# peterdavidfagan/mujoco_robot_environments

Measured on AMD Instinct MI355X. Metric: env steps/sec (whole node), RearrangementEnv batch=4096 at 1/2/4/8 MI355X, higher is better.
Workload: dtype f32

## Files before the change

mujoco_robot_environments_amd/csrc/mre_kernels.hip:

```cpp
#include <hip/hip_runtime.h>

#include "mre_dev.h"
#include "mre_math.h"
#include "mre_collide.h"

namespace mre {
using ModelP = MRE_MODEL_PTR(DevModel);
#if defined(MRE_PHASE_STAMPS) && MRE_PHASE_STAMPS >= 4
__shared__ unsigned long long dbg_acc[4];
#endif

struct OscSm {
  float J[6][7], M[7][7], MiJt[7][6], Li[6][6], Lam[6][6], V[6][6], Jbar[7][6];
  float ep[3], eo[3], F[6], LF[6], tn[7], Jbt[6], xd[6], w[6];
};

struct alignas(8) Blk {
  uint16_t row0;
  uint8_t type, nrows;
  uint8_t rslot;
  uint8_t pa, pb;
  uint8_t primary : 4;
  uint8_t bslot : 4;
};
// ... 1043 lines not shown
        if (ten >= 0) v -= h * grip_bias2 * ten_coef * ten_coef;
      }
    }
    mh_store(s)[e] = v;
#ifdef MRE_NEWTON
    if (i == j) s.scratch[i] = (s.qM[e] - v) * s.qacc[i];
#endif
  }
#ifndef MRE_NEWTON
  if (l < NRV) s.scratch[l] = s.qfrc_smooth[l] + s.qfrc_con[l];
#endif
  MRE_SYNC();
}

MRE_DEV void q_store(float* p, float v) {
  __hip_atomic_store(reinterpret_cast<int*>(p), __float_as_int(v), __ATOMIC_RELAXED, __HIP_MEMORY_SCOPE_AGENT);
}
MRE_DEV void q_store(int* p, int v) { __hip_atomic_store(p, v, __ATOMIC_RELAXED, __HIP_MEMORY_SCOPE_AGENT); }
template <bool WT>
MRE_DEV void travel_store(float* p, float v) {
  if (WT) q_store(p, v); else *p = v;
}
typedef unsigned q_u32x4 __attribute__((ext_vector_type(4)));
MRE_DEV void q_store_row(float* row, const float* src, int n, int l, bool zero_last = false) {
  const __amdgpu_buffer_rsrc_t rsrc = __builtin_amdgcn_make_buffer_rsrc(row, 0, n * 4, 0x00020000);
  if (4 * l < n) {
    q_u32x4 v;
    v.x = __float_as_uint(src[4 * l]); v.y = __float_as_uint(src[4 * l + 1]); v.z = __float_as_uint(src[4 * l + 2]);
    v.w = zero_last && 4 * l + 4 == n ? 0u : __float_as_uint(src[4 * l + 3]);
    __builtin_amdgcn_raw_buffer_store_b128(v, rsrc, 16 * l, 0, 16 );
  }
}

template <bool WT>
MRE_PHASE_FN void integrate(ModelP M, Sm& s, int l, unsigned flags, bool polished, float* clo) {
  const float h = M->opt_rec.timestep;
  const auto* DR = &M->dof_rec[l < NV ? l : 0];
  const int dof_b = DR->body, dof_pid = DR->propid;
  const auto* BR = &M->body_rec[l < NB ? l : 0];
  const int body_qa = BR->qposadr, body_da = BR->dofadr, body_pid = BR->propid;
  const bool freeze = (flags & F_FREEZE_ROBOT) != 0;
  float vl_in = 0.f, ql_in[7] = {0.f, 0.f, 0.f, 0.f, 0.f, 0.f, 0.f};
  if (clo != nullptr) {
    if (l >= NRV && l < NV) vl_in = clo[(QFINE_CUBE_V - QFINE_CUBE_Q) + (l - NRV)];
    if (l >= NRB && l < NB) {
#pragma unroll
      for (int k = 0; k < 7; k++) ql_in[k] = clo[7 * (l - NRB) + k];
    }
  }
  keep_live(dof_pid); keep_live(body_pid); keep_live(body_qa); keep_live(body_da);
  if (l < NV) {
    const int b = dof_b;
    if (b < NRB) {
      if (!freeze) {
#ifdef MRE_NEWTON
        const double acc = polished ? reinterpret_cast<const double*>(&s.nw_Mv[0])[l] : (double)s.qacc[l];
        const double v = robot_v(s, l) + (double)h * (acc + (double)s.scratch[l]);
#else
        const double v = robot_v(s, l) + (double)h * (double)s.scratch[l];
#endif
        const float hi = (float)v;
        s.qvel[l] = hi; s.qlo[QFINE / 2 + l] = (float)(v - (double)hi);
      }
    } else if (prop_is_active(s, dof_pid)) {
      if (clo != nullptr) {
        float* const vl = clo + (QFINE_CUBE_V - QFINE_CUBE_Q) + (l - NRV);
        const double v = (double)s.qvel[l] + (double)vl_in + (double)h * (double)s.qacc[l];
        const float hi = (float)v, lo = (float)(v - (double)hi);
        s.qvel[l] = hi; travel_store<WT>(vl, lo);
        s.scratch[l] = lo;
      } else {
        s.qvel[l] += h * s.qacc[l];
      }
    }
  }
  MRE_SYNC();
  if (l >= 1 && l < NB) {
    const int b = l, qa = body_qa, da = body_da;
    if (b < NRB) {
      if (!freeze) {
        const double q = robot_q(s, qa) + (double)h * robot_v(s, da);
        const float hi = (float)q;
        s.qpos[qa] = hi; s.qlo[qa] = (float)(q - (double)hi);
      }
    } else if (prop_is_active(s, body_pid) && clo != nullptr) {
      float* const ql = clo + 7 * (b - NRB);
      double vv[6];
      for (int k = 0; k < 6; k++) vv[k] = (double)s.qvel[da + k] + (double)s.scratch[da + k];
      for (int k = 0; k < 3; k++) {
        const double x = (double)s.qpos[qa + k] + (double)ql_in[k] + (double)h * vv[k];
        const float hi = (float)x;
        s.qpos[qa + k] = hi; travel_store<WT>(ql + k, (float)(x - (double)hi));
      }
      double q0[4], qn[4];
      for (int k = 0; k < 4; k++) q0[k] = (double)s.qpos[qa + 3 + k] + (double)ql_in[3 + k];
      const double wn2 = vv[3] * vv[3] + vv[4] * vv[4] + vv[5] * vv[5];
      if (wn2 > 1e-60) {
        const double inv = rsq64(wn2), half = 0.5 * (double)h * wn2 * inv;
        double sn, cs;
        sincos_poly_d(half, sn, cs);
        const double ax = vv[3] * inv * sn, ay = vv[4] * inv * sn, az = vv[5] * inv * sn;
        qn[0] = q0[0] * cs - q0[1] * ax - q0[2] * ay - q0[3] * az;
        qn[1] = q0[0] * ax + q0[1] * cs + q0[2] * az - q0[3] * ay;
        qn[2] = q0[0] * ay - q0[1] * az + q0[2] * cs + q0[3] * ax;
        qn[3] = q0[0] * az + q0[1] * ay - q0[2] * ax + q0[3] * cs;
      } else {
        for (int k = 0; k < 4; k++) qn[k] = q0[k];
      }
      const double nn = qn[0] * qn[0] + qn[1] * qn[1] + qn[2] * qn[2] + qn[3] * qn[3];
      const double sc = nn > 1e-30 ? rsq64(nn) : 1.0;
      for (int k = 0; k < 4; k++) {
        const double x = qn[k] * sc;
        const float hi = (float)x;
        s.qpos[qa + 3 + k] = hi; travel_store<WT>(ql + 3 + k, (float)(x - (double)hi));
      }
    } else if (prop_is_active(s, body_pid)) {
      for (int k = 0; k < 3; k++) s.qpos[qa + k] += h * s.qvel[da + k];
      float w[3] = {s.qvel[da + 3], s.qvel[da + 4], s.qvel[da + 5]};
      const float ang = v3normalize(w) * h;
      float qr[4], qn[4], q0[4];
      axisangle2q(qr, w, ang);
      for (int k = 0; k < 4; k++) q0[k] = s.qpos[qa + 3 + k];
      qmul(qn, q0, qr);
      qnormalize(qn);
      for (int k = 0; k < 4; k++) s.qpos[qa + 3 + k] = qn[k];
    }
  }
  MRE_SYNC();
}

#ifdef MRE_PHASE_STAMPS
#define MRE_STAMP(k)                                                         \
  do {                                                                       \
    if ((k) < 12 || MRE_PHASE_STAMPS == 3) {                                 \
      const unsigned long long now_ = __builtin_amdgcn_s_memtime();          \
      if ((k) / 4 == MRE_PHASE_STAMPS) stamp_acc[(k) % 4] += now_ - stamp_t; \
      stamp_t = now_;                                                        \
    }                                                                        \
  } while (0)
#else
#define MRE_STAMP(k) do {} while (0)
#endif

MRE_DEV int q_load(const int* p) { return __hip_atomic_load(p, __ATOMIC_RELAXED, __HIP_MEMORY_SCOPE_AGENT); }

#ifdef MRE_LARGE_CAPS
constexpr bool Q_LARGE = true;
#else
constexpr bool Q_LARGE = false;
#endif
MRE_DEV int* q_bucket(const StepArgs& a, int t, int sh) {
  const int S = a.q_shards;
  return a.q_buf + (size_t)t * a.q_stride + (sh < S ? (size_t)sh * a.q_cap : (size_t)S * a.q_cap + (size_t)(sh - S) * a.q_capl);
}

MRE_DEV int queue_pop_shard(const StepArgs& a, int l, int sh, int& env, int& tick) {
  const int S = a.q_shards;
  const bool order0 = sh < S;
  const int n0 = (a.N - sh + S - 1) / S;
  int* const head = a.q_head + sh * QUEUE_TICKS_MAX;
  const int* const tail = a.q_tail + sh * QUEUE_TICKS_MAX;
  for (;;) {
    int h[QUEUE_TICKS_MAX / 64], tl[QUEUE_TICKS_MAX / 64];
#pragma unroll
    for (int c = 0; c < QUEUE_TICKS_MAX / 64; c++) {
      const int b = c * 64 + l;
      h[c] = 0; tl[c] = 0;
      if (b < a.q_nticks) { h[c] = q_load(head + b); tl[c] = (b == 0 && order0) ? n0 : q_load(tail + b); }
    }
    int t = -1, ht = 0;
#pragma unroll
    for (int c = 0; c < QUEUE_TICKS_MAX / 64; c++) {
      if (t < 0 && c * 64 < a.q_nticks) {
        const unsigned long long ready = __ballot(h[c] < tl[c]);
        if (ready != 0ull) {
          const int k = __ffsll((long long)ready) - 1;
          t = c * 64 + k;
          ht = __builtin_amdgcn_readlane(h[c], k);
        }
      }
    }
    if (t < 0) return 0;
    int got = -1;
    if (l == 0) {
      if (t == 0 && order0) {
        const int i = __hip_atomic_fetch_add(head, 1, __ATOMIC_RELAXED, __HIP_MEMORY_SCOPE_AGENT);
        if (i < n0) got = a.env_order != nullptr ? a.env_order[sh + S * i] : sh + S * i;
      } else {
        int expect = ht;
        if (__hip_atomic_compare_exchange_strong(head + t, &expect, ht + 1, __ATOMIC_RELAXED, __ATOMIC_RELAXED,
                                                 __HIP_MEMORY_SCOPE_AGENT)) {
          const int* slot = q_bucket(a, t, sh) + ht;
          int v = q_load(slot);
          for (unsigned spin = 0; v == 0; ++spin) {
            if (spin > (1u << 20)) { *a.q_err = 1; v = -1; break; }
            __builtin_amdgcn_s_sleep(4);
            v = q_load(slot);
          }
          got = v < 0 ? -2 : v - 1;
        }
      }
    }
    got = __builtin_amdgcn_readfirstlane(got);
    if (got == -2) return -1;
    if (got < 0) continue;
    env = got; tick = t;
    return 1;
  }
}
MRE_DEV bool queue_pop(const StepArgs& a, int l, int home, int& env, int& tick, int& shard, bool wait = true) {
  const int S = a.q_shards;
  if (Q_LARGE) {
    const int SL = a.q_lshards;
    for (unsigned idle = 0;; ++idle) {
      int r = 0;
      for (int k = 0; k < SL && r == 0; ++k) {
        const int sh = S + (home + k < SL ? home + k : home + k - SL);
        r = queue_pop_shard(a, l, sh, env, tick);
        if (r != 0) shard = sh;
      }
      if (r != 0) return r > 0;
      if (!wait || a.q_wait == 0 || q_load(a.q_done) >= a.N) return false;
      if (idle > 512u && q_load(a.q_started) == 0) return false;
      if (idle > (1u << 18)) return false;
      __builtin_amdgcn_s_sleep(127);
    }
  }
  for (int k = 0; k < S; ++k) {
    const int sh = home + k < S ? home + k : home + k - S;
    const int r = queue_pop_shard(a, l, sh, env, tick);
    if (r != 0) { shard = sh; return r > 0; }
  }
  return false;
}
#ifdef MRE_NEWTON
constexpr bool Q_WRITE_THROUGH = true;
#else
constexpr bool Q_WRITE_THROUGH = false;
#endif
MRE_DEV void queue_push(const StepArgs& a, int l, int env, int tick, int shard) {
  if (!Q_WRITE_THROUGH) __builtin_amdgcn_fence(__ATOMIC_RELEASE, "agent");
  asm volatile("s_waitcnt vmcnt(0)" ::: "memory");
  if (l == 0) {
    const int i = __hip_atomic_fetch_add(a.q_tail + shard * QUEUE_TICKS_MAX + tick, 1, __ATOMIC_RELAXED, __HIP_MEMORY_SCOPE_AGENT);
    __hip_atomic_store(q_bucket(a, tick, shard) + i, env + 1, __ATOMIC_RELAXED, __HIP_MEMORY_SCOPE_AGENT);
  }
}

struct QueueItem {
  bool have = false;
  int env = 0, tick = 0, shard = 0, nprops = 0;
  float qpos = 0.f, qvel = 0.f, qacc = 0.f, qfine = 0.f, ctrl = 0.f, prop_size = 0.f;
};
#ifdef MRE_NEWTON
constexpr bool Q_EARLY_TAKE = true;
#else
constexpr bool Q_EARLY_TAKE = false;
#endif
MRE_DEV void queue_take(const StepArgs& a, int l, int home, bool wait, QueueItem& it) {
  it.have = queue_pop(a, l, home, it.env, it.tick, it.shard, wait);
  if (!it.have) return;
  if (it.tick > 0 || Q_LARGE) __builtin_amdgcn_fence(__ATOMIC_ACQUIRE, "agent");
  const size_t e = (size_t)it.env;
  it.qpos = l < NQP ? a.qpos[e * NQP + l] : 0.f;
  it.qvel = l < NVP ? a.qvel[e * NVP + l] : 0.f;
  it.qacc = l < NVP ? a.qacc_ws[e * NVP + l] : 0.f;
  it.qfine = l < QFINE && a.qfine != nullptr ? a.qfine[e * QFINE_ROW + l] : 0.f;
  it.ctrl = l < NU ? a.ctrl[e * NU + l] : 0.f;
  it.prop_size = l < NPROP * 3 ? a.prop_size[e * NPROP * 3 + l] : 0.f;
  it.nprops = a.nprops[e];
}

template <bool QUEUE>
MRE_DEV void step_body(const StepArgs& a, Sm& s) {
  OscSm& osc = s.osc;
  const int l = threadIdx.x;
  int env = 0, qtick = 0, qshard = 0;
  if (!QUEUE) {
    if ((int)blockIdx.x >= a.N) return;
    env = a.env_order != nullptr ? a.env_order[blockIdx.x] : (int)blockIdx.x;
  }
  if (QUEUE && !Q_LARGE && l == 0) __hip_atomic_fetch_add(a.q_started, 1, __ATOMIC_RELAXED, __HIP_MEMORY_SCOPE_AGENT);
  if (QUEUE && Q_LARGE && a.q_wait != 0) {
    for (unsigned idle = 0; q_load(a.q_gen) != a.q_gen_expect; ++idle) {
      if (idle > 1024u) return;
      __builtin_amdgcn_s_sleep(127);
    }
  }
  const int qhome = QUEUE ? (int)(blockIdx.x % (unsigned)(Q_LARGE ? a.q_lshards : a.q_shards)) : 0;
  QueueItem next;
 for (;;) {
  if (QUEUE) {
    if (!next.have) queue_take(a, l, qhome, true, next);
    if (!next.have) return;
    env = next.env; qtick = next.tick; qshard = next.shard;
    next.have = false;
  }
  const int step_lo = QUEUE ? qtick * a.control_steps : 0, step_hi = QUEUE ? step_lo + a.control_steps : a.nsteps;
  if (QUEUE && !Q_LARGE && qtick == 0 && a.large != nullptr && a.large[env] != 0) continue;
  if (!QUEUE || (!Q_LARGE && qtick == 0)) {
#define MRE_PASS_SKIP { if (QUEUE) { if (l == 0) __hip_atomic_fetch_add(a.q_done, 1, __ATOMIC_RELAXED, __HIP_MEMORY_SCOPE_AGENT); continue; } return; }
  if (!QUEUE && a.large != nullptr && (a.large[env] != 0) != (a.want_large != 0)) return;
  if (a.env_mask != nullptr && a.env_mask[env] == 0) {
    if (a.launch_info != nullptr && l < 4) a.launch_info[(size_t)env * 4 + l] = -1;
    MRE_PASS_SKIP;
  }
  if (a.pending != nullptr && a.pending[env] != 0) {
    if (a.launch_info != nullptr && l < 4) a.launch_info[(size_t)env * 4 + l] = l == 0 ? -2 : -1;
    MRE_PASS_SKIP;
  }
#undef MRE_PASS_SKIP
  }
  ModelP M = (ModelP)a.M;

  const bool save = !QUEUE && a.sv_qpos != nullptr && step_lo == 0;
  if (l < NQP) {
    const float v = QUEUE ? next.qpos : a.qpos[(size_t)env * NQP + l];
    s.qpos[l] = v;
    if (save) a.sv_qpos[(size_t)env * NQP + l] = v;
  }
  if (l < NVP) {
    const float v = QUEUE ? next.qvel : a.qvel[(size_t)env * NVP + l], w = QUEUE ? next.qacc : a.qacc_ws[(size_t)env * NVP + l];
    s.qvel[l] = v;
    s.qacc[l] = w;
    s.qfrc_con[l] = 0.f;
    if (save) { a.sv_qvel[(size_t)env * NVP + l] = v; a.sv_qacc_ws[(size_t)env * NVP + l] = w; }
  }
  if (l < QFINE) {
    const float v = QUEUE ? next.qfine : a.qfine != nullptr ? a.qfine[(size_t)env * QFINE_ROW + l] : 0.f;
    s.qlo[l] = v;
    if (save && a.qfine != nullptr) a.sv_qfine[(size_t)env * QFINE_ROW + l] = v;
  }
  if (save && a.qfine != nullptr && l < QFINE_ROW - QFINE)
    a.sv_qfine[(size_t)env * QFINE_ROW + QFINE + l] = a.qfine[(size_t)env * QFINE_ROW + QFINE + l];
  float cube_lo_keep = 0.f;
  if (QUEUE && !Q_LARGE && a.qfine != nullptr && l < QFINE_ROW - QFINE) cube_lo_keep = a.qfine[(size_t)env * QFINE_ROW + QFINE + l];
  if (l < NU) {
    const float v = QUEUE ? next.ctrl : a.ctrl[(size_t)env * NU + l];
    s.ctrl[l] = v;
    if (save) a.sv_ctrl[(size_t)env * NU + l] = v;
  }
  if (save && l == 0) {
    if (a.nstep != nullptr) a.sv_nstep[env] = a.nstep[env];
    a.sv_status[env] = a.status[env];
    a.sv_converged[env] = a.converged != nullptr ? a.converged[env] : (uint8_t)0;
  }
  if (l == 0) { s.nprops = QUEUE ? next.nprops : a.nprops[env]; s.overflow = 0; s.ncon = 0; s.nefc = 0; s.solver_iters = 0; }
#ifdef MRE_NEWTON
  if (l < 24) s.zrow[l] = 0.f;
#endif
  if (l < NPROP * 3) {
    const float sz = QUEUE ? next.prop_size : a.prop_size[(size_t)env * NPROP * 3 + l];
    s.prop_size[l / 3][l % 3] = sz;
  }
  MRE_SYNC();
  if (l < NPROP) {
    const float m = M->body_mass[NRB + l];
    const float* z = s.prop_size[l];
    s.prop_mass[l] = m;
    s.prop_inertia[l][0] = m / 3.f * (z[1] * z[1] + z[2] * z[2]);
    s.prop_inertia[l][1] = m / 3.f * (z[0] * z[0] + z[2] * z[2]);
    s.prop_inertia[l][2] = m / 3.f * (z[0] * z[0] + z[1] * z[1]);
  }
  MRE_SYNC();

#if defined(MRE_PHASE_STAMPS) && MRE_PHASE_STAMPS >= 4
  if (l < 4) dbg_acc[l] = 0ull;
#endif
#ifdef MRE_PHASE_STAMPS
  unsigned long long stamp_acc[4] = {0, 0, 0, 0};
  unsigned long long stamp_t = __builtin_amdgcn_s_memtime();
#endif
  bool arm_converged = ((a.flags & F_CONV_CONTINUE) != 0 || (QUEUE && qtick > 0)) && a.converged != nullptr && a.converged[env] != 0;
  float grip_cmd = 0.f;
  const OscConfig* oscp = a.osc + (size_t)env * a.osc_stride;
  int hw_ncon = 0, hw_nefc = 0, hw_nrrow = 0, hw_npp = 0;
  const unsigned long long launch_t0 = __builtin_amdgcn_s_memtime();
  if (a.mode == CTRL_OSC) {
    if (l < 16) s.osc_tgt[l] = a.osc_target[(size_t)env * 16 + l];
    grip_cmd = a.grip_closed[env] ? M->act_ctrlrange[NU - 1][1] : M->act_ctrlrange[NU - 1][0];
    MRE_SYNC();
  }
  int steps_done = 0;
  bool settled = false;
  for (int step = step_lo; step < step_hi; ++step) {
    MRE_STAMP(7);
    position_stage(M, s, l);
    MRE_STAMP(12);
    MRE_STAMP(13);
    gripper_local(M, s, l);
    if ((a.flags & F_NO_CONSTRAINTS) == 0) connect_rows_local(M, s, l);
    MRE_STAMP(14);
    crb_mass_matrix(M, s, l);
    MRE_SYNC();
#ifndef MRE_NEWTON
    factor_robot_regs(s.qM, s.qLD, s.qLDinv);
#endif
    MRE_STAMP(15);
    MRE_STAMP(0);

    velocity_stage(M, s, l);
    MRE_SYNC();
    finger_bias(M, s, l);
    MRE_STAMP(1);
    const bool constrained = (a.flags & F_NO_CONSTRAINTS) == 0;
    if (constrained) {

      collide(M, s, l, false, (a.flags & F_CLIP_ALWAYS) != 0);
      MRE_STAMP(2);
      assemble_constraints(M, s, l);
#ifdef MRE_NEWTON
      nw_build_lists(s, l, a.flags);
#else
      solve_robot_rows(s, l);
      assemble_blocks(M, s, l);
#endif
      MRE_STAMP(3);
      hw_ncon = max(hw_ncon, s.ncon); hw_nefc = max(hw_nefc, s.nefc);
      hw_nrrow = max(hw_nrrow, s.nrrow); hw_npp = max(hw_npp, s.npp);
    }

    if (a.mode == CTRL_SEQ && (step % a.control_steps) == 0) {
      const int tick = step / a.control_steps;
      if (l < NU) s.ctrl[l] = a.ctrl_seq[((size_t)tick * a.seq_stride + env) * NU + l];
      MRE_SYNC();
    }
    if (a.mode == CTRL_OSC && (step % a.control_steps) == 0) {
      if (step > 0 && osc_converged(M, s, oscp, s.osc_tgt)) arm_converged = true;
      osc_compute(M, s, osc, oscp, s.osc_tgt, l);
      if (l == 0) s.ctrl[NU - 1] = grip_cmd;
      MRE_SYNC();
    }
    MRE_STAMP(4);
    const unsigned clamped = smooth_forces(M, s, l);
    MRE_STAMP(5);
    bool polished = false;
    if (constrained) {
#if defined(MRE_NEWTON) && defined(MRE_PHASE_STAMPS)
      newton_solve(M, s, l, stamp_acc, stamp_t);
      polished = nw_robot_polish(M, s, l);
#elif defined(MRE_NEWTON)
      newton_solve(M, s, l);
      polished = nw_robot_polish(M, s, l);
#else
      if (M->opt_rec.cone == 0) solve_constraints_pyramidal(M, s, l);
      else solve_constraints(M, s, l);
#endif
      MRE_STAMP(6);
    } else {
      if (l < NVP) { s.qacc[l] = s.qacc_smooth[l]; s.qfrc_con[l] = 0.f; }
      MRE_SYNC();
    }

    if (QUEUE && Q_EARLY_TAKE && step + 1 == step_hi) queue_take(a, l, qhome, false, next);
    float cube_lo_warm = 0.f;
    if (QUEUE && Q_WRITE_THROUGH && a.qfine != nullptr && l < QFINE_ROW - QFINE) cube_lo_warm = a.qfine[(size_t)env * QFINE_ROW + QFINE + l];
    integrate_setup(M, s, l, clamped);
    factor_solve_robot(mh_store(s), s.scratch, l);
    if (QUEUE && Q_WRITE_THROUGH) keep_live(cube_lo_warm);
    integrate<QUEUE && Q_WRITE_THROUGH>(M, s, l, a.flags, polished, a.qfine != nullptr ? a.qfine + (size_t)env * QFINE_ROW + QFINE_CUBE_Q : nullptr);
    steps_done = step + 1 - step_lo;
    if ((a.flags & F_SETTLE_EXIT) != 0) {
      float mv = 0.f, ma = 0.f;
      if (l >= NRV && l < NRV + 6 * s.nprops) { mv = fabsf(s.qvel[l]); ma = fabsf(s.qacc[l]); }
      mv = wave_max(mv); ma = wave_max(ma);
      settled = mv < 1e-3f && ma < 1e-2f && step + 1 > a.min_settle_steps;
    }
    if (a.trace != nullptr && env < a.trace_nenv && (a.trace_base + step) < a.trace_max) {
      if (l < TRACE_QVEL) {
        float v = l < NQ ? s.qpos[l] : 0.f;
        if (l == NQ && constrained) {
          int mask = 0;
          for (int k = 0; k < s.nl; k++) mask |= 1 << ((s.lim_info[k] & 0xFF) - 1);
          v = (float)(s.ncon + 64 * mask);
        }
        if (l == NQ + 1 && constrained) {
          unsigned h = 0u;
          for (int c = 0; c < s.ncon; c++) {
            const int pr = s.con_pair[c];
            const unsigned key = (unsigned)(M->pair_g1[pr] * 32 + M->pair_g2[pr] + 1);
            h = (h + key * key) & 0x3FFFFFu;
          }
          v = (float)h;
        }
        if (l == NQ + 2 && constrained && M->opt_rec.cone != 0) {
          unsigned h = 0u;
          const int ns = 7 + s.nl;
          for (int i = 7; i < ns; i++) h += (s.frc[i] > 0.f ? 1u : 2u) * (unsigned)((i + 1) * (i + 1));
          for (int c = 0; c < s.ncon; c++) {
            const int i = ns + 3 * c;
#ifdef MRE_NEWTON
            const float mu = s.con_fric[c];
#else
            const float mu = s.blkrec[8 + c][15];
#endif
            const float fn = s.frc[i], ft2 = s.frc[i + 1] * s.frc[i + 1] + s.frc[i + 2] * s.frc[i + 2], lim = mu * fn;
            const unsigned z = fn <= 0.f ? 1u : (ft2 >= lim * lim * (1.f - 1e-4f) ? 3u : 2u);
            h += z * (unsigned)((c + 3) * (c + 3));
          }
          v = (float)(h & 0x3FFFFFu);
        }
        travel_store<QUEUE && Q_WRITE_THROUGH>(&a.trace[((size_t)(a.trace_base + step) * a.trace_nenv + env) * TRACE_W + l], v);
      }
      if (l < NVP)
        travel_store<QUEUE && Q_WRITE_THROUGH>(&a.trace[((size_t)(a.trace_base + step) * a.trace_nenv + env) * TRACE_W + TRACE_QVEL + l],
                                               l < NV ? s.qvel[l] : 0.f);
    }
    if (settled) break;
  }
  MRE_STAMP(7);
  if (a.settle_steps != nullptr && l == 0) a.settle_steps[env] = settled ? steps_done : -steps_done;
  const bool hand_over = QUEUE && !Q_LARGE && s.overflow != 0;
  if (QUEUE && Q_WRITE_THROUGH) {
    if (hand_over) {
      if (a.qfine != nullptr && l < QFINE_ROW - QFINE) q_store(a.qfine + (size_t)env * QFINE_ROW + QFINE + l, cube_lo_keep);
    } else {
      q_store_row(a.qpos + (size_t)env * NQP, s.qpos, NQP, l);
      q_store_row(a.qvel + (size_t)env * NVP, s.qvel, NVP, l);
      q_store_row(a.qacc_ws + (size_t)env * NVP, s.qacc, NVP, l, true);
      if (a.qfine != nullptr) q_store_row(a.qfine + (size_t)env * QFINE_ROW, s.qlo, QFINE, l);
      q_store_row(a.ctrl + (size_t)env * NU, s.ctrl, NU, l);
    }
  }
  if (a.nstep != nullptr && l == 0 && !hand_over) {
    if (QUEUE) __hip_atomic_fetch_add(a.nstep + env, steps_done, __ATOMIC_RELAXED, __HIP_MEMORY_SCOPE_AGENT);
    else a.nstep[env] += steps_done;
  }
  if (a.nsteps == 0 && (a.flags & F_OSC_EVAL) != 0 && a.mode == CTRL_OSC) {
    position_stage(M, s, l);
    gripper_local(M, s, l);
    crb_mass_matrix(M, s, l);
    MRE_SYNC();
    velocity_stage(M, s, l);
    MRE_SYNC();
    osc_compute(M, s, osc, oscp, s.osc_tgt, l);
    if (l == 0) s.ctrl[NU - 1] = grip_cmd;
    MRE_SYNC();
  }
  if (a.nsteps == 0 && (a.flags & F_DETECT) != 0 && a.contacts != nullptr) {
    position_stage(M, s, l);
    collide(M, s, l, (a.flags & F_DETECT_ACTIVE) == 0, (a.flags & F_CLIP_ALWAYS) != 0);
    float* o = a.contacts + (size_t)env * (1 + 3 * CONTACT_EXPORT);
    const int n = s.ncon < CONTACT_EXPORT ? s.ncon : CONTACT_EXPORT;
    if (l == 0) o[0] = s.overflow ? -(float)s.ncon : (float)s.ncon;
    if (l < n) {
      const int pr = s.con_pair[l];
      o[1 + 3 * l] = (float)M->pair_g1[pr]; o[2 + 3 * l] = (float)M->pair_g2[pr]; o[3 + 3 * l] = s.con_dist[l];
      if (a.contacts_full != nullptr) {
        float* f = a.contacts_full + ((size_t)env * CONTACT_EXPORT + l) * 12;
        for (int k = 0; k < 3; k++) f[k] = s.con_pos[l][k];
        for (int k = 0; k < 9; k++) f[3 + k] = s.con_frame[l][k];
      }
    }
    MRE_SYNC();
    if (l == 0) s.overflow = 0;
  }
  const bool q_last = !QUEUE || (qtick + 1 == a.q_nticks && !hand_over);
  if (q_last && (a.mode == CTRL_OSC || a.sites != nullptr || a.geoms != nullptr)) kinematics_only(M, s, l);
  if (a.mode == CTRL_OSC && a.nsteps > 0 && !hand_over) {
    if (q_last && osc_converged(M, s, oscp, s.osc_tgt)) arm_converged = true;
    if (l == 0) {
      if (a.converged != nullptr) {
        if (QUEUE && Q_WRITE_THROUGH) __hip_atomic_store(a.converged + env, (uint8_t)(arm_converged ? 1 : 0), __ATOMIC_RELAXED, __HIP_MEMORY_SCOPE_AGENT);
        else a.converged[env] = arm_converged ? 1 : 0;
      }
      if (q_last && !arm_converged && a.status != nullptr && (a.flags & F_CONV_OPEN) == 0) {
        if (QUEUE) __hip_atomic_fetch_or(a.status + env, 1u, __ATOMIC_RELAXED, __HIP_MEMORY_SCOPE_AGENT);
        else a.status[env] |= 1u;
      }
    }
  }
  if (a.geoms != nullptr && l < NG) {
    float p[3], R[9], size[3], rb;
    geom_pose(M, s, l, p, R, size, &rb);
    float* o = a.geoms + ((size_t)env * NG + l) * 16;
    const int pid = M->geom_propid[l];
    const bool active = pid < 0 || pid < s.nprops;
    for (int k = 0; k < 3; k++) o[k] = p[k];
    for (int k = 0; k < 9; k++) o[3 + k] = R[k];
    for (int k = 0; k < 3; k++) o[12 + k] = size[k];
    o[15] = active ? (float)M->geom_type[l] : -1.f;
  }
  if (a.sites != nullptr && q_last) {
    float* o = a.sites + (size_t)env * 16;
    if (l < 3) o[l] = s.site_xpos[M->opt_rec.tcp_site][l];
    if (l >= 3 && l < 6) o[l] = s.site_xpos[M->opt_rec.eef_site][l - 3];
    if (l == 6) {
      float q[4];
      mat2q(q, s.site_xmat[0]);
      o[6] = q[0]; o[7] = q[1]; o[8] = q[2]; o[9] = q[3];
    }
  }
  if (QUEUE && Q_WRITE_THROUGH) {
  } else if (hand_over) {
    if (a.qfine != nullptr && l < QFINE_ROW - QFINE) a.qfine[(size_t)env * QFINE_ROW + QFINE + l] = cube_lo_keep;
  } else {
    if (l < NQP) a.qpos[(size_t)env * NQP + l] = s.qpos[l];
    if (l < NVP) {
      a.qvel[(size_t)env * NVP + l] = s.qvel[l];
      a.qacc_ws[(size_t)env * NVP + l] = l < NV ? s.qacc[l] : 0.f;
    }
    if (l < QFINE && a.qfine != nullptr) a.qfine[(size_t)env * QFINE_ROW + l] = s.qlo[l];
    if (l < NU) a.ctrl[(size_t)env * NU + l] = s.ctrl[l];
  }
  const bool q_more = QUEUE && !hand_over && qtick + 1 < a.q_nticks;
  if (l == 0 && a.launch_info != nullptr) {
    int* li = a.launch_info + (size_t)env * 4;
    unsigned long long dt = (__builtin_amdgcn_s_memtime() - launch_t0) >> 10;
    int moved = 0;
    if (QUEUE) {
      int* qa = a.q_acc + (size_t)env * 4;
      if (qtick > 0 || Q_LARGE) {
        hw_ncon = max(hw_ncon, q_load(qa + 0) & 0xFFFF); hw_nefc = max(hw_nefc, q_load(qa + 1));
        hw_nrrow = max(hw_nrrow, q_load(qa + 2) & 0xFFFF); hw_npp = max(hw_npp, q_load(qa + 2) >> 16);
        dt += (unsigned long long)q_load(qa + 3);
        moved = q_load(qa + 0) >> 16;
      }
      if (hand_over) moved = 1;
      if ((q_more || hand_over) && Q_WRITE_THROUGH) {
        q_store(qa + 0, hw_ncon | (moved << 16)); q_store(qa + 1, hw_nefc); q_store(qa + 2, hw_nrrow | (hw_npp << 16)); q_store(qa + 3, (int)dt);
      } else if (q_more || hand_over) {
        qa[0] = hw_ncon | (moved << 16); qa[1] = hw_nefc; qa[2] = hw_nrrow | (hw_npp << 16); qa[3] = (int)dt;
      }
      else dt /= (unsigned long long)(qtick + 1);
    }
    if (!q_more && !hand_over) {
#ifdef MRE_LARGE_CAPS
      li[0] = (s.overflow ? 2 : 0) | (moved ? 4 : 0);
#else
      li[0] = s.overflow ? 1 : 0;
#endif
      li[1] = hw_ncon | ((int)(dt < 0x7FFFull ? dt : 0x7FFFull) << 16); li[2] = hw_nefc; li[3] = hw_nrrow | (hw_npp << 16);
    }
  }
#ifndef MRE_LARGE_CAPS
  if (!QUEUE && l == 0 && a.pending != nullptr && s.overflow) a.pending[env] = 1;
#endif
  if (l == 0 && a.status != nullptr && !hand_over) {
    unsigned st = 0;
    for (int k = 0; k < NQ; k++) if (!isfinite(s.qpos[k])) st |= 2u;
    if (s.overflow) st |= 4u;
    if (QUEUE) { if (st) __hip_atomic_fetch_or(a.status + env, st, __ATOMIC_RELAXED, __HIP_MEMORY_SCOPE_AGENT); }
    else a.status[env] |= st;
    if (a.stats != nullptr && a.nsteps > 0 && !(QUEUE && Q_WRITE_THROUGH && q_more)) {
      a.stats[env * 4 + 0] = s.ncon; a.stats[env * 4 + 1] = s.nefc;
      a.stats[env * 4 + 2] = s.solver_iters; a.stats[env * 4 + 3] = s.nl;
#ifdef MRE_PHASE_STAMPS
      for (int k = 0; k < 4; k++) a.stats[env * 4 + k] = (int)(stamp_acc[k] >> 4);
#if MRE_PHASE_STAMPS >= 4
      for (int k = 0; k < 4; k++) a.stats[env * 4 + k] = (int)(dbg_acc[k] >> 4);
#endif
#endif
    }
  }
  if (!QUEUE) return;
  if (hand_over) queue_push(a, l, env, qtick, a.q_shards + env % a.q_lshards);
  else if (q_more) queue_push(a, l, env, qtick + 1, qshard);
  else if (l == 0) __hip_atomic_fetch_add(a.q_done, 1, __ATOMIC_RELAXED, __HIP_MEMORY_SCOPE_AGENT);
 }
}

#ifdef MRE_NEWTON
#define MRE_VARIANT(name) name##_newton
#else
#define MRE_VARIANT(name) name
#endif

#ifdef MRE_LARGE_CAPS
__global__ __launch_bounds__(64, 2) void MRE_VARIANT(k_step_large)(StepArgs a) {
  __shared__ Sm s;
  step_body<false>(a, s);
}
}

extern "C" void MRE_VARIANT(mre_launch_step_large)(const mre::StepArgs* args, hipStream_t stream) {
  hipLaunchKernelGGL(mre::MRE_VARIANT(k_step_large), dim3(args->N), dim3(64), 0, stream, *args);
}
namespace mre {
__global__ __launch_bounds__(64, 2) void MRE_VARIANT(k_step_queue_large)(StepArgs a) {
  __shared__ Sm s;
  step_body<true>(a, s);
}
}
extern "C" void MRE_VARIANT(mre_launch_step_queue_large)(const mre::StepArgs* args, int nwaves, hipStream_t stream) {
  hipLaunchKernelGGL(mre::MRE_VARIANT(k_step_queue_large), dim3(nwaves), dim3(64), 0, stream, *args);
}
#else
__global__ __launch_bounds__(64, 2) void MRE_VARIANT(k_step)(StepArgs a) {
  __shared__ Sm s;
  step_body<false>(a, s);
}
// ... 366 lines not shown
```

Measured before the change: 25.99 million.

## Load cold kernel args lazily and keep cube low words in LDS, not global

Rarely used StepArgs fields are now read on demand from the kernarg segment through volatile loads, so the compiler stops holding them in scalar registers across the long step loop. The cubes' low-order position and velocity words are kept in a register per lane and staged through shared memory borrowed from the constraint block during integration. This replaces the per-step global or atomic write-through to qfine, which is now written once at the end. The aim is to cut SGPR pressure and per-step global traffic. The cost is extra kernarg reloads at the use sites and an added barrier in integrate.

```diff
diff --git a/mujoco_robot_environments_amd/csrc/mre_kernels.hip b/mujoco_robot_environments_amd/csrc/mre_kernels.hip
--- a/mujoco_robot_environments_amd/csrc/mre_kernels.hip
+++ b/mujoco_robot_environments_amd/csrc/mre_kernels.hip
@@ -1099,8 +1099,14 @@
   }
 }
 
-template <bool WT>
-MRE_PHASE_FN void integrate(ModelP M, Sm& s, int l, unsigned flags, bool polished, float* clo) {
+MRE_DEV float* cube_lo_room(Sm& s) { return &s.JpA[0][0]; }
+static_assert(sizeof(((Sm*)0)->JpA) >= sizeof(float) * (QFINE_ROW - QFINE) && QFINE_ROW - QFINE <= 64, "the cubes' low words fit the head of the constraint block, one per lane");
+MRE_PHASE_FN float integrate(ModelP M, Sm& s, int l, unsigned flags, bool polished, bool have_lo, float cube_lo) {
+  float* const clo = cube_lo_room(s);
+  if (have_lo) {
+    if (l < QFINE_ROW - QFINE) clo[l] = cube_lo;
+    MRE_SYNC();
+  }
   const float h = M->opt_rec.timestep;
   const auto* DR = &M->dof_rec[l < NV ? l : 0];
   const int dof_b = DR->body, dof_pid = DR->propid;
@@ -1108,7 +1114,7 @@
   const int body_qa = BR->qposadr, body_da = BR->dofadr, body_pid = BR->propid;
   const bool freeze = (flags & F_FREEZE_ROBOT) != 0;
   float vl_in = 0.f, ql_in[7] = {0.f, 0.f, 0.f, 0.f, 0.f, 0.f, 0.f};
-  if (clo != nullptr) {
+  if (have_lo) {
     if (l >= NRV && l < NV) vl_in = clo[(QFINE_CUBE_V - QFINE_CUBE_Q) + (l - NRV)];
     if (l >= NRB && l < NB) {
 #pragma unroll
@@ -1130,11 +1136,11 @@
         s.qvel[l] = hi; s.qlo[QFINE / 2 + l] = (float)(v - (double)hi);
       }
     } else if (prop_is_active(s, dof_pid)) {
-      if (clo != nullptr) {
+      if (have_lo) {
         float* const vl = clo + (QFINE_CUBE_V - QFINE_CUBE_Q) + (l - NRV);
         const double v = (double)s.qvel[l] + (double)vl_in + (double)h * (double)s.qacc[l];
         const float hi = (float)v, lo = (float)(v - (double)hi);
-        s.qvel[l] = hi; travel_store<WT>(vl, lo);
+        s.qvel[l] = hi; *vl = lo;
         s.scratch[l] = lo;
       } else {
         s.qvel[l] += h * s.qacc[l];
@@ -1150,14 +1156,14 @@
         const float hi = (float)q;
         s.qpos[qa] = hi; s.qlo[qa] = (float)(q - (double)hi);
       }
-    } else if (prop_is_active(s, body_pid) && clo != nullptr) {
+    } else if (prop_is_active(s, body_pid) && have_lo) {
       float* const ql = clo + 7 * (b - NRB);
       double vv[6];
       for (int k = 0; k < 6; k++) vv[k] = (double)s.qvel[da + k] + (double)s.scratch[da + k];
       for (int k = 0; k < 3; k++) {
         const double x = (double)s.qpos[qa + k] + (double)ql_in[k] + (double)h * vv[k];
         const float hi = (float)x;
-        s.qpos[qa + k] = hi; travel_store<WT>(ql + k, (float)(x - (double)hi));
+        s.qpos[qa + k] = hi; ql[k] = (float)(x - (double)hi);
       }
       double q0[4], qn[4];
       for (int k = 0; k < 4; k++) q0[k] = (double)s.qpos[qa + 3 + k] + (double)ql_in[3 + k];
@@ -1179,7 +1185,7 @@
       for (int k = 0; k < 4; k++) {
         const double x = qn[k] * sc;
         const float hi = (float)x;
-        s.qpos[qa + 3 + k] = hi; travel_store<WT>(ql + 3 + k, (float)(x - (double)hi));
+        s.qpos[qa + 3 + k] = hi; ql[3 + k] = (float)(x - (double)hi);
       }
     } else if (prop_is_active(s, body_pid)) {
       for (int k = 0; k < 3; k++) s.qpos[qa + k] += h * s.qvel[da + k];
@@ -1194,6 +1200,8 @@
     }
   }
   MRE_SYNC();
+  if (have_lo && l < QFINE_ROW - QFINE) cube_lo = clo[l];
+  return cube_lo;
 }
 
 #ifdef MRE_PHASE_STAMPS
@@ -1211,6 +1219,18 @@
 
 MRE_DEV int q_load(const int* p) { return __hip_atomic_load(p, __ATOMIC_RELAXED, __HIP_MEMORY_SCOPE_AGENT); }
 
+#if defined(__HIP_DEVICE_COMPILE__)
+template <class T>
+MRE_DEV T cold_arg(size_t off) {
+  const char __attribute__((address_space(4)))* seg = (const char __attribute__((address_space(4)))*)__builtin_amdgcn_kernarg_segment_ptr();
+  return *(const volatile T __attribute__((address_space(4)))*)(seg + off);
+}
+#else
+template <class T>
+MRE_DEV T cold_arg(size_t) { return T(); }
+#endif
+#define MRE_COLD(member) cold_arg<decltype(StepArgs::member)>(offsetof(StepArgs, member))
+
 #ifdef MRE_LARGE_CAPS
 constexpr bool Q_LARGE = true;
 #else
@@ -1252,7 +1272,7 @@
     if (l == 0) {
       if (t == 0 && order0) {
         const int i = __hip_atomic_fetch_add(head, 1, __ATOMIC_RELAXED, __HIP_MEMORY_SCOPE_AGENT);
-        if (i < n0) got = a.env_order != nullptr ? a.env_order[sh + S * i] : sh + S * i;
+        if (i < n0) { const int* const order = MRE_COLD(env_order); got = order != nullptr ? order[sh + S * i] : sh + S * i; }
       } else {
         int expect = ht;
         if (__hip_atomic_compare_exchange_strong(head + t, &expect, ht + 1, __ATOMIC_RELAXED, __ATOMIC_RELAXED,
@@ -1260,7 +1280,7 @@
           const int* slot = q_bucket(a, t, sh) + ht;
           int v = q_load(slot);
           for (unsigned spin = 0; v == 0; ++spin) {
-            if (spin > (1u << 20)) { *a.q_err = 1; v = -1; break; }
+            if (spin > (1u << 20)) { *MRE_COLD(q_err) = 1; v = -1; break; }
             __builtin_amdgcn_s_sleep(4);
             v = q_load(slot);
           }
@@ -1287,8 +1307,8 @@
         if (r != 0) shard = sh;
       }
       if (r != 0) return r > 0;
-      if (!wait || a.q_wait == 0 || q_load(a.q_done) >= a.N) return false;
-      if (idle > 512u && q_load(a.q_started) == 0) return false;
+      if (!wait || MRE_COLD(q_wait) == 0 || q_load(MRE_COLD(q_done)) >= a.N) return false;
+      if (idle > 512u && q_load(MRE_COLD(q_started)) == 0) return false;
       if (idle > (1u << 18)) return false;
       __builtin_amdgcn_s_sleep(127);
     }
@@ -1317,7 +1337,7 @@
 struct QueueItem {
   bool have = false;
   int env = 0, tick = 0, shard = 0, nprops = 0;
-  float qpos = 0.f, qvel = 0.f, qacc = 0.f, qfine = 0.f, ctrl = 0.f, prop_size = 0.f;
+  float qpos = 0.f, qvel = 0.f, qacc = 0.f, qfine = 0.f, cube_lo = 0.f, ctrl = 0.f, prop_size = 0.f;
 };
 #ifdef MRE_NEWTON
 constexpr bool Q_EARLY_TAKE = true;
@@ -1333,6 +1353,7 @@
   it.qvel = l < NVP ? a.qvel[e * NVP + l] : 0.f;
   it.qacc = l < NVP ? a.qacc_ws[e * NVP + l] : 0.f;
   it.qfine = l < QFINE && a.qfine != nullptr ? a.qfine[e * QFINE_ROW + l] : 0.f;
+  it.cube_lo = l < QFINE_ROW - QFINE && a.qfine != nullptr ? a.qfine[e * QFINE_ROW + QFINE + l] : 0.f;
   it.ctrl = l < NU ? a.ctrl[e * NU + l] : 0.f;
   it.prop_size = l < NPROP * 3 ? a.prop_size[e * NPROP * 3 + l] : 0.f;
   it.nprops = a.nprops[e];
@@ -1345,11 +1366,14 @@
   int env = 0, qtick = 0, qshard = 0;
   if (!QUEUE) {
     if ((int)blockIdx.x >= a.N) return;
-    env = a.env_order != nullptr ? a.env_order[blockIdx.x] : (int)blockIdx.x;
-  }
-  if (QUEUE && !Q_LARGE && l == 0) __hip_atomic_fetch_add(a.q_started, 1, __ATOMIC_RELAXED, __HIP_MEMORY_SCOPE_AGENT);
-  if (QUEUE && Q_LARGE && a.q_wait != 0) {
-    for (unsigned idle = 0; q_load(a.q_gen) != a.q_gen_expect; ++idle) {
+    const int* const order = MRE_COLD(env_order);
+    env = order != nullptr ? order[blockIdx.x] : (int)blockIdx.x;
+  }
+  if (QUEUE && !Q_LARGE && l == 0) __hip_atomic_fetch_add(MRE_COLD(q_started), 1, __ATOMIC_RELAXED, __HIP_MEMORY_SCOPE_AGENT);
+  if (QUEUE && Q_LARGE && MRE_COLD(q_wait) != 0) {
+    const int* const gen = MRE_COLD(q_gen);
+    const int gen_expect = MRE_COLD(q_gen_expect);
+    for (unsigned idle = 0; q_load(gen) != gen_expect; ++idle) {
       if (idle > 1024u) return;
       __builtin_amdgcn_s_sleep(127);
     }
@@ -1364,53 +1388,67 @@
     next.have = false;
   }
   const int step_lo = QUEUE ? qtick * a.control_steps : 0, step_hi = QUEUE ? step_lo + a.control_steps : a.nsteps;
-  if (QUEUE && !Q_LARGE && qtick == 0 && a.large != nullptr && a.large[env] != 0) continue;
+  if (QUEUE && !Q_LARGE && qtick == 0) {
+    const uint8_t* const large = MRE_COLD(large);
+    if (large != nullptr && large[env] != 0) continue;
+  }
   if (!QUEUE || (!Q_LARGE && qtick == 0)) {
-#define MRE_PASS_SKIP { if (QUEUE) { if (l == 0) __hip_atomic_fetch_add(a.q_done, 1, __ATOMIC_RELAXED, __HIP_MEMORY_SCOPE_AGENT); continue; } return; }
-  if (!QUEUE && a.large != nullptr && (a.large[env] != 0) != (a.want_large != 0)) return;
-  if (a.env_mask != nullptr && a.env_mask[env] == 0) {
-    if (a.launch_info != nullptr && l < 4) a.launch_info[(size_t)env * 4 + l] = -1;
+#define MRE_PASS_SKIP { if (QUEUE) { if (l == 0) __hip_atomic_fetch_add(MRE_COLD(q_done), 1, __ATOMIC_RELAXED, __HIP_MEMORY_SCOPE_AGENT); continue; } return; }
+  if (!QUEUE) {
+    const uint8_t* const large = MRE_COLD(large);
+    if (large != nullptr && (large[env] != 0) != (MRE_COLD(want_large) != 0)) return;
+  }
+  const uint8_t* const env_mask = MRE_COLD(env_mask);
+  if (env_mask != nullptr && env_mask[env] == 0) {
+    int* const info = MRE_COLD(launch_info);
+    if (info != nullptr && l < 4) info[(size_t)env * 4 + l] = -1;
     MRE_PASS_SKIP;
   }
-  if (a.pending != nullptr && a.pending[env] != 0) {
-    if (a.launch_info != nullptr && l < 4) a.launch_info[(size_t)env * 4 + l] = l == 0 ? -2 : -1;
+  const uint8_t* const pending = MRE_COLD(pending);
+  if (pending != nullptr && pending[env] != 0) {
+    int* const info = MRE_COLD(launch_info);
+    if (info != nullptr && l < 4) info[(size_t)env * 4 + l] = l == 0 ? -2 : -1;
     MRE_PASS_SKIP;
   }
 #undef MRE_PASS_SKIP
   }
   ModelP M = (ModelP)a.M;
 
-  const bool save = !QUEUE && a.sv_qpos != nullptr && step_lo == 0;
+  const bool save = !QUEUE && MRE_COLD(sv_qpos) != nullptr && step_lo == 0;
   if (l < NQP) {
     const float v = QUEUE ? next.qpos : a.qpos[(size_t)env * NQP + l];
     s.qpos[l] = v;
-    if (save) a.sv_qpos[(size_t)env * NQP + l] = v;
+    if (save) MRE_COLD(sv_qpos)[(size_t)env * NQP + l] = v;
   }
   if (l < NVP) {
     const float v = QUEUE ? next.qvel : a.qvel[(size_t)env * NVP + l], w = QUEUE ? next.qacc : a.qacc_ws[(size_t)env * NVP + l];
     s.qvel[l] = v;
     s.qacc[l] = w;
     s.qfrc_con[l] = 0.f;
-    if (save) { a.sv_qvel[(size_t)env * NVP + l] = v; a.sv_qacc_ws[(size_t)env * NVP + l] = w; }
+    if (save) { MRE_COLD(sv_qvel)[(size_t)env * NVP + l] = v; MRE_COLD(sv_qacc_ws)[(size_t)env * NVP + l] = w; }
   }
   if (l < QFINE) {
     const float v = QUEUE ? next.qfine : a.qfine != nullptr ? a.qfine[(size_t)env * QFINE_ROW + l] : 0.f;
     s.qlo[l] = v;
-    if (save && a.qfine != nullptr) a.sv_qfine[(size_t)env * QFINE_ROW + l] = v;
-  }
-  if (save && a.qfine != nullptr && l < QFINE_ROW - QFINE)
-    a.sv_qfine[(size_t)env * QFINE_ROW + QFINE + l] = a.qfine[(size_t)env * QFINE_ROW + QFINE + l];
-  float cube_lo_keep = 0.f;
-  if (QUEUE && !Q_LARGE && a.qfine != nullptr && l < QFINE_ROW - QFINE) cube_lo_keep = a.qfine[(size_t)env * QFINE_ROW + QFINE + l];
+    if (save && a.qfine != nullptr) MRE_COLD(sv_qfine)[(size_t)env * QFINE_ROW + l] = v;
+  }
+  const bool have_lo = a.qfine != nullptr;
+  float cube_lo = 0.f;
+  if (l < QFINE_ROW - QFINE && have_lo) {
+    cube_lo = QUEUE ? next.cube_lo : a.qfine[(size_t)env * QFINE_ROW + QFINE + l];
+    if (save) MRE_COLD(sv_qfine)[(size_t)env * QFINE_ROW + QFINE + l] = cube_lo;
+  }
   if (l < NU) {
     const float v = QUEUE ? next.ctrl : a.ctrl[(size_t)env * NU + l];
     s.ctrl[l] = v;
-    if (save) a.sv_ctrl[(size_t)env * NU + l] = v;
+    if (save) MRE_COLD(sv_ctrl)[(size_t)env * NU + l] = v;
   }
   if (save && l == 0) {
-    if (a.nstep != nullptr) a.sv_nstep[env] = a.nstep[env];
-    a.sv_status[env] = a.status[env];
-    a.sv_converged[env] = a.converged != nullptr ? a.converged[env] : (uint8_t)0;
+    const int* const nstep = MRE_COLD(nstep);
+    const uint8_t* const converged = MRE_COLD(converged);
+    if (nstep != nullptr) MRE_COLD(sv_nstep)[env] = nstep[env];
+    MRE_COLD(sv_status)[env] = MRE_COLD(status)[env];
+    MRE_COLD(sv_converged)[env] = converged != nullptr ? converged[env] : (uint8_t)0;
   }
   if (l == 0) { s.nprops = QUEUE ? next.nprops : a.nprops[env]; s.overflow = 0; s.ncon = 0; s.nefc = 0; s.solver_iters = 0; }
 #ifdef MRE_NEWTON
@@ -1438,18 +1476,23 @@
   unsigned long long stamp_acc[4] = {0, 0, 0, 0};
   unsigned long long stamp_t = __builtin_amdgcn_s_memtime();
 #endif
-  bool arm_converged = ((a.flags & F_CONV_CONTINUE) != 0 || (QUEUE && qtick > 0)) && a.converged != nullptr && a.converged[env] != 0;
+  bool arm_converged = false;
+  if ((a.flags & F_CONV_CONTINUE) != 0 || (QUEUE && qtick > 0)) {
+    const uint8_t* const converged = MRE_COLD(converged);
+    arm_converged = converged != nullptr && converged[env] != 0;
+  }
   float grip_cmd = 0.f;
-  const OscConfig* oscp = a.osc + (size_t)env * a.osc_stride;
+  const auto osc_of = [](int e) { return MRE_COLD(osc) + (size_t)e * MRE_COLD(osc_stride); };
   int hw_ncon = 0, hw_nefc = 0, hw_nrrow = 0, hw_npp = 0;
   const unsigned long long launch_t0 = __builtin_amdgcn_s_memtime();
   if (a.mode == CTRL_OSC) {
-    if (l < 16) s.osc_tgt[l] = a.osc_target[(size_t)env * 16 + l];
-    grip_cmd = a.grip_closed[env] ? M->act_ctrlrange[NU - 1][1] : M->act_ctrlrange[NU - 1][0];
+    if (l < 16) s.osc_tgt[l] = MRE_COLD(osc_target)[(size_t)env * 16 + l];
+    grip_cmd = MRE_COLD(grip_closed)[env] ? M->act_ctrlrange[NU - 1][1] : M->act_ctrlrange[NU - 1][0];
     MRE_SYNC();
   }
   int steps_done = 0;
   bool settled = false;
+  const bool tracing = MRE_COLD(trace) != nullptr;
   for (int step = step_lo; step < step_hi; ++step) {
     MRE_STAMP(7);
     position_stage(M, s, l);
@@ -1493,6 +1536,7 @@
       MRE_SYNC();
     }
     if (a.mode == CTRL_OSC && (step % a.control_steps) == 0) {
+      const OscConfig* const oscp = osc_of(env);
       if (step > 0 && osc_converged(M, s, oscp, s.osc_tgt)) arm_converged = true;
       osc_compute(M, s, osc, oscp, s.osc_tgt, l);
       if (l == 0) s.ctrl[NU - 1] = grip_cmd;
@@ -1520,20 +1564,19 @@
     }
 
     if (QUEUE && Q_EARLY_TAKE && step + 1 == step_hi) queue_take(a, l, qhome, false, next);
-    float cube_lo_warm = 0.f;
-    if (QUEUE && Q_WRITE_THROUGH && a.qfine != nullptr && l < QFINE_ROW - QFINE) cube_lo_warm = a.qfine[(size_t)env * QFINE_ROW + QFINE + l];
     integrate_setup(M, s, l, clamped);
     factor_solve_robot(mh_store(s), s.scratch, l);
-    if (QUEUE && Q_WRITE_THROUGH) keep_live(cube_lo_warm);
-    integrate<QUEUE && Q_WRITE_THROUGH>(M, s, l, a.flags, polished, a.qfine != nullptr ? a.qfine + (size_t)env * QFINE_ROW + QFINE_CUBE_Q : nullptr);
+    cube_lo = integrate(M, s, l, a.flags, polished, have_lo, cube_lo);
     steps_done = step + 1 - step_lo;
     if ((a.flags & F_SETTLE_EXIT) != 0) {
       float mv = 0.f, ma = 0.f;
       if (l >= NRV && l < NRV + 6 * s.nprops) { mv = fabsf(s.qvel[l]); ma = fabsf(s.qacc[l]); }
       mv = wave_max(mv); ma = wave_max(ma);
-      settled = mv < 1e-3f && ma < 1e-2f && step + 1 > a.min_settle_steps;
-    }
-    if (a.trace != nullptr && env < a.trace_nenv && (a.trace_base + step) < a.trace_max) {
+      settled = mv < 1e-3f && ma < 1e-2f && step + 1 > MRE_COLD(min_settle_steps);
+    }
+    float* const trace = tracing ? MRE_COLD(trace) : nullptr;
+    const int trace_nenv = tracing ? MRE_COLD(trace_nenv) : 0, trace_base = tracing ? MRE_COLD(trace_base) : 0;
+    if (tracing && env < trace_nenv && (trace_base + step) < MRE_COLD(trace_max)) {
       if (l < TRACE_QVEL) {
         float v = l < NQ ? s.qpos[l] : 0.f;
         if (l == NQ && constrained) {
@@ -1567,54 +1610,66 @@
           }
           v = (float)(h & 0x3FFFFFu);
         }
-        travel_store<QUEUE && Q_WRITE_THROUGH>(&a.trace[((size_t)(a.trace_base + step) * a.trace_nenv + env) * TRACE_W + l], v);
+        travel_store<QUEUE && Q_WRITE_THROUGH>(&trace[((size_t)(trace_base + step) * trace_nenv + env) * TRACE_W + l], v);
       }
       if (l < NVP)
-        travel_store<QUEUE && Q_WRITE_THROUGH>(&a.trace[((size_t)(a.trace_base + step) * a.trace_nenv + env) * TRACE_W + TRACE_QVEL + l],
+        travel_store<QUEUE && Q_WRITE_THROUGH>(&trace[((size_t)(trace_base + step) * trace_nenv + env) * TRACE_W + TRACE_QVEL + l],
                                                l < NV ? s.qvel[l] : 0.f);
     }
     if (settled) break;
   }
   MRE_STAMP(7);
-  if (a.settle_steps != nullptr && l == 0) a.settle_steps[env] = settled ? steps_done : -steps_done;
+  int* const settle_steps = MRE_COLD(settle_steps);
+  int* const nstep = MRE_COLD(nstep);
+  const int nsteps = MRE_COLD(nsteps);
+  float* const sites = MRE_COLD(sites);
+  float* const geoms = MRE_COLD(geoms);
+  uint32_t* const status = MRE_COLD(status);
+  int* const launch_info = MRE_COLD(launch_info);
+  int* const stats = MRE_COLD(stats);
+#ifndef MRE_LARGE_CAPS
+  uint8_t* const pending_w = QUEUE ? nullptr : MRE_COLD(pending);
+#endif
   const bool hand_over = QUEUE && !Q_LARGE && s.overflow != 0;
   if (QUEUE && Q_WRITE_THROUGH) {
-    if (hand_over) {
-      if (a.qfine != nullptr && l < QFINE_ROW - QFINE) q_store(a.qfine + (size_t)env * QFINE_ROW + QFINE + l, cube_lo_keep);
-    } else {
+    if (!hand_over) {
       q_store_row(a.qpos + (size_t)env * NQP, s.qpos, NQP, l);
       q_store_row(a.qvel + (size_t)env * NVP, s.qvel, NVP, l);
       q_store_row(a.qacc_ws + (size_t)env * NVP, s.qacc, NVP, l, true);
       if (a.qfine != nullptr) q_store_row(a.qfine + (size_t)env * QFINE_ROW, s.qlo, QFINE, l);
+      if (have_lo && steps_done > 0 && l < QFINE_ROW - QFINE) q_store(a.qfine + (size_t)env * QFINE_ROW + QFINE + l, cube_lo);
       q_store_row(a.ctrl + (size_t)env * NU, s.ctrl, NU, l);
     }
   }
-  if (a.nstep != nullptr && l == 0 && !hand_over) {
-    if (QUEUE) __hip_atomic_fetch_add(a.nstep + env, steps_done, __ATOMIC_RELAXED, __HIP_MEMORY_SCOPE_AGENT);
-    else a.nstep[env] += steps_done;
-  }
-  if (a.nsteps == 0 && (a.flags & F_OSC_EVAL) != 0 && a.mode == CTRL_OSC) {
+  if (settle_steps != nullptr && l == 0) settle_steps[env] = settled ? steps_done : -steps_done;
+  if (nstep != nullptr && l == 0 && !hand_over) {
+    if (QUEUE) __hip_atomic_fetch_add(nstep + env, steps_done, __ATOMIC_RELAXED, __HIP_MEMORY_SCOPE_AGENT);
+    else nstep[env] += steps_done;
+  }
+  if (nsteps == 0 && (a.flags & F_OSC_EVAL) != 0 && a.mode == CTRL_OSC) {
     position_stage(M, s, l);
     gripper_local(M, s, l);
     crb_mass_matrix(M, s, l);
     MRE_SYNC();
     velocity_stage(M, s, l);
     MRE_SYNC();
-    osc_compute(M, s, osc, oscp, s.osc_tgt, l);
+    osc_compute(M, s, osc, osc_of(env), s.osc_tgt, l);
     if (l == 0) s.ctrl[NU - 1] = grip_cmd;
     MRE_SYNC();
   }
-  if (a.nsteps == 0 && (a.flags & F_DETECT) != 0 && a.contacts != nullptr) {
+  float* const contacts = nsteps == 0 && (a.flags & F_DETECT) != 0 ? MRE_COLD(contacts) : nullptr;
+  if (contacts != nullptr) {
     position_stage(M, s, l);
     collide(M, s, l, (a.flags & F_DETECT_ACTIVE) == 0, (a.flags & F_CLIP_ALWAYS) != 0);
-    float* o = a.contacts + (size_t)env * (1 + 3 * CONTACT_EXPORT);
+    float* o = contacts + (size_t)env * (1 + 3 * CONTACT_EXPORT);
+    float* const contacts_full = MRE_COLD(contacts_full);
     const int n = s.ncon < CONTACT_EXPORT ? s.ncon : CONTACT_EXPORT;
     if (l == 0) o[0] = s.overflow ? -(float)s.ncon : (float)s.ncon;
     if (l < n) {
       const int pr = s.con_pair[l];
       o[1 + 3 * l] = (float)M->pair_g1[pr]; o[2 + 3 * l] = (float)M->pair_g2[pr]; o[3 + 3 * l] = s.con_dist[l];
-      if (a.contacts_full != nullptr) {
-        float* f = a.contacts_full + ((size_t)env * CONTACT_EXPORT + l) * 12;
+      if (contacts_full != nullptr) {
+        float* f = contacts_full + ((size_t)env * CONTACT_EXPORT + l) * 12;
         for (int k = 0; k < 3; k++) f[k] = s.con_pos[l][k];
         for (int k = 0; k < 9; k++) f[3 + k] = s.con_frame[l][k];
       }
@@ -1623,24 +1678,25 @@
     if (l == 0) s.overflow = 0;
   }
   const bool q_last = !QUEUE || (qtick + 1 == a.q_nticks && !hand_over);
-  if (q_last && (a.mode == CTRL_OSC || a.sites != nullptr || a.geoms != nullptr)) kinematics_only(M, s, l);
-  if (a.mode == CTRL_OSC && a.nsteps > 0 && !hand_over) {
-    if (q_last && osc_converged(M, s, oscp, s.osc_tgt)) arm_converged = true;
+  if (q_last && (a.mode == CTRL_OSC || sites != nullptr || geoms != nullptr)) kinematics_only(M, s, l);
+  if (a.mode == CTRL_OSC && nsteps > 0 && !hand_over) {
+    if (q_last && osc_converged(M, s, osc_of(env), s.osc_tgt)) arm_converged = true;
+    uint8_t* const converged = MRE_COLD(converged);
     if (l == 0) {
-      if (a.converged != nullptr) {
-        if (QUEUE && Q_WRITE_THROUGH) __hip_atomic_store(a.converged + env, (uint8_t)(arm_converged ? 1 : 0), __ATOMIC_RELAXED, __HIP_MEMORY_SCOPE_AGENT);
-        else a.converged[env] = arm_converged ? 1 : 0;
+      if (converged != nullptr) {
+        if (QUEUE && Q_WRITE_THROUGH) __hip_atomic_store(converged + env, (uint8_t)(arm_converged ? 1 : 0), __ATOMIC_RELAXED, __HIP_MEMORY_SCOPE_AGENT);
+        else converged[env] = arm_converged ? 1 : 0;
       }
-      if (q_last && !arm_converged && a.status != nullptr && (a.flags & F_CONV_OPEN) == 0) {
-        if (QUEUE) __hip_atomic_fetch_or(a.status + env, 1u, __ATOMIC_RELAXED, __HIP_MEMORY_SCOPE_AGENT);
-        else a.status[env] |= 1u;
+      if (q_last && !arm_converged && status != nullptr && (a.flags & F_CONV_OPEN) == 0) {
+        if (QUEUE) __hip_atomic_fetch_or(status + env, 1u, __ATOMIC_RELAXED, __HIP_MEMORY_SCOPE_AGENT);
+        else status[env] |= 1u;
       }
     }
   }
-  if (a.geoms != nullptr && l < NG) {
+  if (geoms != nullptr && l < NG) {
     float p[3], R[9], size[3], rb;
     geom_pose(M, s, l, p, R, size, &rb);
-    float* o = a.geoms + ((size_t)env * NG + l) * 16;
+    float* o = geoms + ((size_t)env * NG + l) * 16;
     const int pid = M->geom_propid[l];
     const bool active = pid < 0 || pid < s.nprops;
     for (int k = 0; k < 3; k++) o[k] = p[k];
@@ -1648,8 +1704,8 @@
     for (int k = 0; k < 3; k++) o[12 + k] = size[k];
     o[15] = active ? (float)M->geom_type[l] : -1.f;
   }
-  if (a.sites != nullptr && q_last) {
-    float* o = a.sites + (size_t)env * 16;
+  if (sites != nullptr && q_last) {
+    float* o = sites + (size_t)env * 16;
     if (l < 3) o[l] = s.site_xpos[M->opt_rec.tcp_site][l];
     if (l >= 3 && l < 6) o[l] = s.site_xpos[M->opt_rec.eef_site][l - 3];
     if (l == 6) {
@@ -1659,24 +1715,23 @@
     }
   }
   if (QUEUE && Q_WRITE_THROUGH) {
-  } else if (hand_over) {
-    if (a.qfine != nullptr && l < QFINE_ROW - QFINE) a.qfine[(size_t)env * QFINE_ROW + QFINE + l] = cube_lo_keep;
-  } else {
+  } else if (!hand_over) {
     if (l < NQP) a.qpos[(size_t)env * NQP + l] = s.qpos[l];
     if (l < NVP) {
       a.qvel[(size_t)env * NVP + l] = s.qvel[l];
       a.qacc_ws[(size_t)env * NVP + l] = l < NV ? s.qacc[l] : 0.f;
     }
     if (l < QFINE && a.qfine != nullptr) a.qfine[(size_t)env * QFINE_ROW + l] = s.qlo[l];
+    if (have_lo && steps_done > 0 && l < QFINE_ROW - QFINE) a.qfine[(size_t)env * QFINE_ROW + QFINE + l] = cube_lo;
     if (l < NU) a.ctrl[(size_t)env * NU + l] = s.ctrl[l];
   }
   const bool q_more = QUEUE && !hand_over && qtick + 1 < a.q_nticks;
-  if (l == 0 && a.launch_info != nullptr) {
-    int* li = a.launch_info + (size_t)env * 4;
+  if (l == 0 && launch_info != nullptr) {
+    int* li = launch_info + (size_t)env * 4;
     unsigned long long dt = (__builtin_amdgcn_s_memtime() - launch_t0) >> 10;
     int moved = 0;
     if (QUEUE) {
-      int* qa = a.q_acc + (size_t)env * 4;
+      int* qa = MRE_COLD(q_acc) + (size_t)env * 4;
       if (qtick > 0 || Q_LARGE) {
         hw_ncon = max(hw_ncon, q_load(qa + 0) & 0xFFFF); hw_nefc = max(hw_nefc, q_load(qa + 1));
         hw_nrrow = max(hw_nrrow, q_load(qa + 2) & 0xFFFF); hw_npp = max(hw_npp, q_load(qa + 2) >> 16);
@@ -1701,21 +1756,21 @@
     }
   }
 #ifndef MRE_LARGE_CAPS
-  if (!QUEUE && l == 0 && a.pending != nullptr && s.overflow) a.pending[env] = 1;
-#endif
-  if (l == 0 && a.status != nullptr && !hand_over) {
+  if (!QUEUE && l == 0 && pending_w != nullptr && s.overflow) pending_w[env] = 1;
+#endif
+  if (l == 0 && status != nullptr && !hand_over) {
     unsigned st = 0;
     for (int k = 0; k < NQ; k++) if (!isfinite(s.qpos[k])) st |= 2u;
     if (s.overflow) st |= 4u;
-    if (QUEUE) { if (st) __hip_atomic_fetch_or(a.status + env, st, __ATOMIC_RELAXED, __HIP_MEMORY_SCOPE_AGENT); }
-    else a.status[env] |= st;
-    if (a.stats != nullptr && a.nsteps > 0 && !(QUEUE && Q_WRITE_THROUGH && q_more)) {
-      a.stats[env * 4 + 0] = s.ncon; a.stats[env * 4 + 1] = s.nefc;
-      a.stats[env * 4 + 2] = s.solver_iters; a.stats[env * 4 + 3] = s.nl;
+    if (QUEUE) { if (st) __hip_atomic_fetch_or(status + env, st, __ATOMIC_RELAXED, __HIP_MEMORY_SCOPE_AGENT); }
+    else status[env] |= st;
+    if (stats != nullptr && nsteps > 0 && !(QUEUE && Q_WRITE_THROUGH && q_more)) {
+      stats[env * 4 + 0] = s.ncon; stats[env * 4 + 1] = s.nefc;
+      stats[env * 4 + 2] = s.solver_iters; stats[env * 4 + 3] = s.nl;
 #ifdef MRE_PHASE_STAMPS
-      for (int k = 0; k < 4; k++) a.stats[env * 4 + k] = (int)(stamp_acc[k] >> 4);
+      for (int k = 0; k < 4; k++) stats[env * 4 + k] = (int)(stamp_acc[k] >> 4);
 #if MRE_PHASE_STAMPS >= 4
-      for (int k = 0; k < 4; k++) a.stats[env * 4 + k] = (int)(dbg_acc[k] >> 4);
+      for (int k = 0; k < 4; k++) stats[env * 4 + k] = (int)(dbg_acc[k] >> 4);
 #endif
 #endif
     }
@@ -1723,7 +1778,7 @@
   if (!QUEUE) return;
   if (hand_over) queue_push(a, l, env, qtick, a.q_shards + env % a.q_lshards);
   else if (q_more) queue_push(a, l, env, qtick + 1, qshard);
-  else if (l == 0) __hip_atomic_fetch_add(a.q_done, 1, __ATOMIC_RELAXED, __HIP_MEMORY_SCOPE_AGENT);
+  else if (l == 0) __hip_atomic_fetch_add(MRE_COLD(q_done), 1, __ATOMIC_RELAXED, __HIP_MEMORY_SCOPE_AGENT);
  }
 }
 
```

After: 26.07 million, median of 6. About the same (+0.3%).
